# mit-han-lab/distrifuser

Hardware: NVIDIA H100
Metric: SDXL 50-step latency (ms/image) (lower is better)
Workload: dtype f16

## Files before the change

### distrifuser_b200/csrc/attention.cu

```cuda

#include "tc_ptx.cuh"

using namespace df;
using namespace df::tc;

namespace {

constexpr int BM = 128;
constexpr int BN = 128;
constexpr int HB = 64;
constexpr int NCONSUMER_WARPS = 8;
constexpr int NTHREADS = 32 * (NCONSUMER_WARPS + 1);
constexpr int WARP_TMA = NCONSUMER_WARPS;
constexpr uint32_t BLK_BYTES = BN * HB * 2;

template <int NBLK, int KSTAGES, int VSTAGES>
struct __align__(1024) SmemT {
  __half q[NBLK][BM * HB];
  __half k[KSTAGES][NBLK][BN * HB];
  __half v[VSTAGES][NBLK][BN * HB];
  uint64_t q_full, q_empty;
  uint64_t k_full[KSTAGES], k_empty[KSTAGES], v_full[VSTAGES], v_empty[VSTAGES];
  uint64_t sched_full[2];
  int sched_code[2];
  uint32_t ticket;
};
template <int NBLK> struct Cfg;
template <> struct Cfg<1> { static constexpr int KST = 3, VST = 2, SN = 128; };
template <> struct Cfg<2> { static constexpr int KST = 2, VST = 2, SN = 64; };
template <> struct Cfg<3> { static constexpr int KST = 2, VST = 1, SN = 64; };

struct Sched {
  int a, R, P;
  int dyn;
  int units;
};
constexpr int ITEM_END = -1;

__device__ __forceinline__ float2 ld_f2(const float2* p) {
  float2 r;
  asm volatile("ld.global.v2.f32 {%0, %1}, [%2];" : "=f"(r.x), "=f"(r.y) : "l"(p) : "memory");
  return r;
}

struct SegInfo {
  int32_t rank[DF_MAX_WORLD];
};

#ifndef DF_EMU_GROUPS
#define DF_EMU_GROUPS 3
#endif

template <int N>
__device__ __forceinline__ void wgmma_ss(float* d, uint64_t a_desc, uint64_t b_desc, uint32_t accumulate) {
  if constexpr (N == 64) wgmma_ss_n64(d, a_desc, b_desc, accumulate);
  else wgmma_ss_n128(d, a_desc, b_desc, accumulate);
}

template <int NBLK>
__global__ void __launch_bounds__(NTHREADS, 1)
fmha_fwd_kernel(const __grid_constant__ CUtensorMap tm_q, const __grid_constant__ CUtensorMap tm_kv_own,
                const CUtensorMap* __restrict__ kvmaps, df_comm_t comm, SegInfo segs, __half* __restrict__ out, int lq,
                int lseg, int heads, int d, int64_t o_pitch, int nseg, int own_seg, int idx, int wait_flags,
                float scale_log2, Sched sched, float* part_o, float2* part_ml, unsigned int* part_cnt, unsigned int* sched_ctr) {
  constexpr int KSTAGES = Cfg<NBLK>::KST, VSTAGES = Cfg<NBLK>::VST;
  constexpr uint32_t TILE_BYTES = NBLK * BLK_BYTES;
  constexpr int SN = Cfg<NBLK>::SN, NSUB = BN / SN;
  using Smem = SmemT<NBLK, KSTAGES, VSTAGES>;
  extern __shared__ __align__(1024) uint8_t smem_raw[];
  Smem& sm = *reinterpret_cast<Smem*>(smem_raw);
  if ((smem_u32(smem_raw) & 1023u) != 0) __trap();

  const int warp = threadIdx.x >> 5, lane = threadIdx.x & 31;
  const int nqt = (lq + BM - 1) / BM;
  const int tps = (lseg + BN - 1) / BN;
  const int T_all = nseg * tps;
  const int n_items = sched.a + ((int)blockIdx.x < sched.R * sched.P ? 1 : 0);
  auto decode = [&](int it, int& q0, int& head, int& bat, int& j_begin, int& T, int& slot, int& lo) {
    int u;
    if (sched.dyn) {
      u = it; j_begin = 0; T = T_all; slot = -1; lo = -1;
    } else if (it < sched.a) {
      u = it * (int)gridDim.x + (int)blockIdx.x; j_begin = 0; T = T_all; slot = -1; lo = -1;
    } else {
      lo = (int)blockIdx.x / sched.P;
      const int part = (int)blockIdx.x - lo * sched.P;
      u = sched.a * (int)gridDim.x + lo;
      j_begin = (int)((long long)part * T_all / sched.P);
      T = (int)((long long)(part + 1) * T_all / sched.P) - j_begin;
      slot = sched.P > 1 ? (int)blockIdx.x : -1;
    }
    const int qt = u % nqt, rest = u / nqt;
    head = rest % heads;
    bat = rest / heads;
    q0 = qt * BM;
  };

  if (threadIdx.x == 0) {
    mbar_init(&sm.q_full, 1);
    mbar_init(&sm.q_empty, NCONSUMER_WARPS);
    for (int s = 0; s < KSTAGES; ++s) { mbar_init(&sm.k_full[s], 1); mbar_init(&sm.k_empty[s], NCONSUMER_WARPS); }
    for (int s = 0; s < VSTAGES; ++s) { mbar_init(&sm.v_full[s], 1); mbar_init(&sm.v_empty[s], NCONSUMER_WARPS); }
    mbar_init(&sm.sched_full[0], 1);
    mbar_init(&sm.sched_full[1], 1);
    asm volatile("fence.mbarrier_init.release.cluster;" ::: "memory");
  }
  __syncthreads();
  pdl_wait();

  if (warp == WARP_TMA) {
    if (lane == 0) {
      prefetch_tmap(&tm_q);
      prefetch_tmap(&tm_kv_own);
      uint32_t rd = 0;
      if (nseg > 1) rd = comm.clock[1];
      int it_static = 0;
      auto draw = [&]() -> unsigned int {
        if (sched.dyn) return atomicAdd(sched_ctr, 1u);
        return (unsigned int)it_static++;
      };
      const unsigned int n_fresh = sched.dyn ? (unsigned int)sched.units : (unsigned int)n_items;
      unsigned int next_t = draw();
      uint32_t g = 0;
      for (uint32_t ui = 0;; ++ui) {
        int code = ITEM_END;
        if (next_t < n_fresh) {
          code = (int)next_t;
          next_t = draw();
        } else if (sched.dyn && next_t == n_fresh + gridDim.x - 1u) {
          *sched_ctr = 0u;
        }
        mbar_wait(&sm.q_empty, (ui & 1u) ^ 1u);
        *(volatile int*)&sm.sched_code[ui & 1u] = code;
        mbar_arrive(&sm.sched_full[ui & 1u]);
        if (code == ITEM_END) break;
        int q0, head, bat, j_begin, T, slot, lo;
        decode(code, q0, head, bat, j_begin, T, slot, lo);
        mbar_expect_tx(&sm.q_full, TILE_BYTES);
#pragma unroll
        for (int blk = 0; blk < NBLK; ++blk) tma_load_4d(sm.q[blk], &tm_q, &sm.q_full, blk * HB, head, q0, bat);
        int so = j_begin / tps, t = j_begin - so * tps;
        for (int j = 0; j < T; ++j, ++t, ++g) {
          if (t == tps) { t = 0; ++so; }
          int seg = own_seg + so;
          if (seg >= nseg) seg -= nseg;
          const void* map = &tm_kv_own;
          if (seg != own_seg) {
            const int r = segs.rank[seg];
            if ((t == 0 || j == 0) && wait_flags) {
              spin_until(flag_ptr(comm, comm.rank, idx, r), rd, comm.spin_timeout_ns);
              asm volatile("fence.proxy.async.global;" ::: "memory");
            }
            map = kvmaps + (size_t)(rd % DF_NBANKS) * comm.world + r;
          }
          const uint32_t ks = g % KSTAGES, vs = g % VSTAGES;
          mbar_wait(&sm.k_empty[ks], ((g / KSTAGES) & 1u) ^ 1u);
          mbar_expect_tx(&sm.k_full[ks], TILE_BYTES);
#pragma unroll
          for (int blk = 0; blk < NBLK; ++blk) tma_load_4d(sm.k[ks][blk], map, &sm.k_full[ks], blk * HB, head, t * BN, bat);
          mbar_wait(&sm.v_empty[vs], ((g / VSTAGES) & 1u) ^ 1u);
          mbar_expect_tx(&sm.v_full[vs], TILE_BYTES);
#pragma unroll
          for (int blk = 0; blk < NBLK; ++blk) tma_load_4d(sm.v[vs][blk], map, &sm.v_full[vs], blk * HB, heads + head, t * BN, bat);
        }
      }
    }
  } else {
    const int wg = warp >> 2;
    const int c4 = lane & 3;
    const int rowA = wg * 64 + (warp & 3) * 16 + (lane >> 2);
    const uint32_t q_base = smem_u32(sm.q) + wg * 64 * 128;
    uint32_t g = 0;
    for (uint32_t ui = 0;; ++ui) {
      mbar_wait(&sm.sched_full[ui & 1u], (ui >> 1) & 1u);
      const int code = *(volatile int*)&sm.sched_code[ui & 1u];
      if (code == ITEM_END) break;
      int q0, head, bat, j_begin, T, slot, lo;
      decode(code, q0, head, bat, j_begin, T, slot, lo);
      float nA = INFINITY, nB = INFINITY;
      float lA = 0.f, lB = 0.f;
      float o[NBLK * 32];
#pragma unroll
      for (int i = 0; i < NBLK * 32; ++i) o[i] = 0.f;
      mbar_wait(&sm.q_full, ui & 1u);
      int t = j_begin % tps;
      for (int j = 0; j < T; ++j, ++t, ++g) {
        if (t == tps) t = 0;
        const int valid = min(BN, lseg - t * BN);
        const uint32_t ks = g % KSTAGES, vs = g % VSTAGES;
#pragma unroll
        for (int sub = 0; sub < NSUB; ++sub) {
          float s[SN / 2];
          if (sub == 0) mbar_wait(&sm.k_full[ks], (g / KSTAGES) & 1u);
          const uint32_t k_addr = smem_u32(sm.k[ks]) + sub * SN * 128;
          wgmma_fence();
#pragma unroll
          for (int blk = 0; blk < NBLK; ++blk)
#pragma unroll
            for (int kk = 0; kk < HB / 16; ++kk)
              wgmma_ss<SN>(s, smem_desc(q_base + blk * BLK_BYTES + kk * 32, 16, 1024), smem_desc(k_addr + blk * BLK_BYTES + kk * 32, 16, 1024),
                           (blk | kk) > 0);
          wgmma_commit();
          wgmma_wait<0>();
          fence_regs<SN / 2>(s);
          if (sub == NSUB - 1) {
            __syncwarp();
            if (lane == 0) {
              mbar_arrive(&sm.k_empty[ks]);
              if (j + 1 == T) mbar_arrive(&sm.q_empty);
            }
          }
          const int vcols = valid - sub * SN;
          if (vcols < SN) {
#pragma unroll
            for (int i = 0; i < SN / 8; ++i)
#pragma unroll
              for (int k = 0; k < 2; ++k)
                if (8 * i + 2 * c4 + k >= vcols) { s[4 * i + k] = -INFINITY; s[4 * i + 2 + k] = -INFINITY; }
          }
          float mA0 = -INFINITY, mA1 = -INFINITY, mB0 = -INFINITY, mB1 = -INFINITY;
#pragma unroll
          for (int i = 0; i < SN / 8; i += 2) {
            mA0 = fmaxf(mA0, fmaxf(s[4 * i], s[4 * i + 1]));
            mB0 = fmaxf(mB0, fmaxf(s[4 * i + 2], s[4 * i + 3]));
            mA1 = fmaxf(mA1, fmaxf(s[4 * i + 4], s[4 * i + 5]));
            mB1 = fmaxf(mB1, fmaxf(s[4 * i + 6], s[4 * i + 7]));
          }
          float mA = fmaxf(mA0, mA1), mB = fmaxf(mB0, mB1);
          mA = fmaxf(mA, __shfl_xor_sync(0xffffffffu, mA, 1));
          mB = fmaxf(mB, __shfl_xor_sync(0xffffffffu, mB, 1));
          mA = fmaxf(mA, __shfl_xor_sync(0xffffffffu, mA, 2));
          mB = fmaxf(mB, __shfl_xor_sync(0xffffffffu, mB, 2));
          const float dA = fmaf(mA, scale_log2, nA), dB = fmaf(mB, scale_log2, nB);
          if (dA > 8.f) {
            const float alpha = ex2(-dA);
            nA = -mA * scale_log2; lA *= alpha;
#pragma unroll
            for (int i = 0; i < NBLK * 8; ++i) { o[4 * i] *= alpha; o[4 * i + 1] *= alpha; }
          }
          if (dB > 8.f) {
            const float alpha = ex2(-dB);
            nB = -mB * scale_log2; lB *= alpha;
#pragma unroll
            for (int i = 0; i < NBLK * 8; ++i) { o[4 * i + 2] *= alpha; o[4 * i + 3] *= alpha; }
          }
          uint32_t pk[SN / 4];
#pragma unroll
          for (int i = 0; i < SN / 8; ++i) {
            const int grp = sub * (SN / 8) + i;
            float e[4];
#pragma unroll
            for (int k = 0; k < 4; ++k) {
              const float x = fmaf(s[4 * i + k], scale_log2, k < 2 ? nA : nB);
              e[k] = ((grp * DF_EMU_GROUPS) / 16 != ((grp + 1) * DF_EMU_GROUPS) / 16) ? ex2_poly(x) : ex2(x);
            }
            lA += e[0] + e[1];
            lB += e[2] + e[3];
            pk[2 * i] = pack_h2(e[0], e[1]);
            pk[2 * i + 1] = pack_h2(e[2], e[3]);
          }
          if (sub == 0) mbar_wait(&sm.v_full[vs], (g / VSTAGES) & 1u);
          const uint32_t v_addr = smem_u32(sm.v[vs]) + sub * SN * 128;
          wgmma_fence();
#pragma unroll
          for (int kk = 0; kk < SN / 16; ++kk)
#pragma unroll
            for (int blk = 0; blk < NBLK; ++blk)
              wgmma_rs_n64(o + 32 * blk, pk + 4 * kk, smem_desc(v_addr + blk * BLK_BYTES + kk * 2048, 16384, 1024), 1u);
          wgmma_commit();
          wgmma_wait<0>();
          fence_regs<NBLK * 32>(o);
        }
        __syncwarp();
        if (lane == 0) mbar_arrive(&sm.v_empty[vs]);
      }
      lA += __shfl_xor_sync(0xffffffffu, lA, 1); lB += __shfl_xor_sync(0xffffffffu, lB, 1);
      lA += __shfl_xor_sync(0xffffffffu, lA, 2); lB += __shfl_xor_sync(0xffffffffu, lB, 2);
      const bool partial = slot >= 0;
      bool finish = !partial;
      float denA = lA, denB = lB;
      if (partial) {
        const int64_t prow = (int64_t)slot * BM + rowA;
        if (c4 == 0) { part_ml[prow] = make_float2(-nA, lA); part_ml[prow + 8] = make_float2(-nB, lB); }
#pragma unroll
        for (int i = 0; i < NBLK * 8; ++i) {
          const int col = 8 * i + 2 * c4;
          *reinterpret_cast<float2*>(part_o + prow * (NBLK * HB) + col) = make_float2(o[4 * i], o[4 * i + 1]);
          *reinterpret_cast<float2*>(part_o + (prow + 8) * (NBLK * HB) + col) = make_float2(o[4 * i + 2], o[4 * i + 3]);
        }
        __threadfence();
        asm volatile("bar.sync 1, 256;" ::: "memory");
        if (threadIdx.x == 0) {
          const unsigned int tk = atomicAdd(part_cnt + lo, 1u);
          sm.ticket = tk;
          if (tk == (unsigned int)sched.P - 1) part_cnt[lo] = 0;
        }
        asm volatile("bar.sync 1, 256;" ::: "memory");
        finish = sm.ticket == (unsigned int)sched.P - 1;
        if (finish) {
          __threadfence();
          const int s0 = lo * sched.P;
#pragma unroll
          for (int h = 0; h < 2; ++h) {
            const int64_t r = rowA + 8 * h;
            float m_max = -INFINITY;
            for (int pp = 0; pp < sched.P; ++pp) m_max = fmaxf(m_max, ld_f2(part_ml + (int64_t)(s0 + pp) * BM + r).x);
            float den = 0.f;
#pragma unroll
            for (int i = 0; i < NBLK * 8; ++i) { o[4 * i + 2 * h] = 0.f; o[4 * i + 2 * h + 1] = 0.f; }
            for (int pp = 0; pp < sched.P; ++pp) {
              const float2 ml = ld_f2(part_ml + (int64_t)(s0 + pp) * BM + r);
              const float w = ex2(ml.x - m_max);
              den = fmaf(w, ml.y, den);
              const float2* src = reinterpret_cast<const float2*>(part_o + ((int64_t)(s0 + pp) * BM + r) * (NBLK * HB));
#pragma unroll
              for (int i = 0; i < NBLK * 8; ++i) {
                const float2 v = ld_f2(src + 4 * i + c4);
                o[4 * i + 2 * h] = fmaf(w, v.x, o[4 * i + 2 * h]);
                o[4 * i + 2 * h + 1] = fmaf(w, v.y, o[4 * i + 2 * h + 1]);
              }
            }
            if (h == 0) denA = den; else denB = den;
          }
        }
      }
      if (finish) {
#pragma unroll
        for (int h = 0; h < 2; ++h) {
          const int row = rowA + 8 * h;
          if (q0 + row >= lq) continue;
          const float inv = 1.f / (h == 0 ? denA : denB);
          __half* dst = out + ((int64_t)bat * lq + q0 + row) * o_pitch + (int64_t)head * d;
#pragma unroll
          for (int i = 0; i < NBLK * 8; ++i) {
            const int col = 8 * i + 2 * c4;
            if (col < d)
              *reinterpret_cast<uint32_t*>(dst + col) = pack_h2(o[4 * i + 2 * h] * inv, o[4 * i + 2 * h + 1] * inv);
          }
        }
      }
    }
  }
}


int make_map(CUtensorMap* m, const void* base, int d, int nheads, int rows, int batch, int64_t pitch) {
  EncodeTiledFn enc = tensor_map_encoder();
  DF_REQUIRE(enc != nullptr, "cuTensorMapEncodeTiled is not available from this driver");
  cuuint64_t dims[4] = {(cuuint64_t)d, (cuuint64_t)nheads, (cuuint64_t)rows, (cuuint64_t)batch};
  cuuint64_t strides[3] = {(cuuint64_t)d * 2, (cuuint64_t)pitch * 2, (cuuint64_t)rows * pitch * 2};
  cuuint32_t box[4] = {HB, 1, BN, 1};
  cuuint32_t estr[4] = {1, 1, 1, 1};
  CUresult r = enc(m, CU_TENSOR_MAP_DATA_TYPE_FLOAT16, 4, const_cast<void*>(base), dims, strides, box, estr,
                   CU_TENSOR_MAP_INTERLEAVE_NONE, CU_TENSOR_MAP_SWIZZLE_128B, CU_TENSOR_MAP_L2_PROMOTION_L2_256B,
                   CU_TENSOR_MAP_FLOAT_OOB_FILL_NONE);
  DF_REQUIRE(r == CUDA_SUCCESS, "cuTensorMapEncodeTiled failed (%d): base=%p d=%d heads=%d rows=%d batch=%d pitch=%lld", (int)r,
             base, d, nheads, rows, batch, (long long)pitch);
  return 0;
}

}

extern "C" int df_attn_make_kvmaps(df_comm_t comm, uint64_t tensor_off, uint64_t slot_bytes, int b, int lseg, int heads,
                                   int d, void* maps_out, void* stream) {
  static_assert(sizeof(CUtensorMap) == DF_TENSORMAP_BYTES, "tensor map size");
  DF_REQUIRE(d % 8 == 0 && d >= 8 && d <= 192, "df_attn: head dim %d not supported (multiple of 8, <= 192)", d);
  DF_REQUIRE(slot_bytes >= (uint64_t)b * lseg * 2 * heads * d * 2, "df_attn_make_kvmaps: slot too small");
  CUtensorMap host[DF_NBANKS * DF_MAX_WORLD];
  memset(host, 0, sizeof(host));
  const int64_t pitch = 2 * (int64_t)heads * d;
  for (int k = 0; k < DF_NBANKS; ++k)
    for (int s = 0; s < comm.world; ++s) {
      const char* base = slot_ptr(comm, comm.rank, (uint32_t)k, tensor_off, slot_bytes, s);
      if (int rc = make_map(&host[k * comm.world + s], base, d, 2 * heads, lseg, b, pitch)) return rc;
    }
  DF_CHECK_CUDA(cudaMemcpyAsync(maps_out, host, sizeof(CUtensorMap) * DF_NBANKS * comm.world, cudaMemcpyHostToDevice,
                                (cudaStream_t)stream));
  DF_CHECK_CUDA(cudaStreamSynchronize((cudaStream_t)stream));
  return 0;
}

namespace {
#ifndef DF_MIN_PART_TILES
#define DF_MIN_PART_TILES 8
#endif
void plan_schedule(int b, int lq, int lseg, int nseg, int heads, int d, bool have_ws, int& grid, Sched& sc) {
  (void)d;
  const long long slots = sm_count();
  const long long units = (long long)((lq + BM - 1) / BM) * heads * b;
  const int t_all = nseg * ((lseg + BN - 1) / BN);
  sc.units = (int)units;
  if (units >= slots) {
    grid = (int)slots;
    sc.a = (int)(units / slots);
    sc.R = (int)(units % slots);
    sc.P = 1;
    sc.dyn = have_ws ? 1 : 0;
  } else {
    long long p = have_ws ? slots / units : 1;
    if (p > t_all / DF_MIN_PART_TILES) p = t_all / DF_MIN_PART_TILES;
    if (p < 1) p = 1;
    sc.a = 0; sc.R = (int)units; sc.P = (int)p; sc.dyn = 0;
    grid = (int)(units * p);
  }
}
constexpr size_t WS_HEADER = 1024;
size_t workspace_need(const Sched& sc, int d) {
  if (sc.P <= 1) return WS_HEADER;
  const size_t hd_pad = (size_t)((d + HB - 1) / HB) * HB;
  const size_t parts = (size_t)sc.R * sc.P;
  return WS_HEADER + 1024 + ((size_t)sc.R * sizeof(unsigned int) + 255) / 256 * 256 + parts * BM * sizeof(float2) + parts * BM * hd_pad * sizeof(float);
}
}

extern "C" size_t df_attn_workspace_bytes(int b, int lq, int lseg, int nseg, int heads, int d) {
  int grid;
  Sched sc;
  plan_schedule(b, lq, lseg, nseg, heads, d, true, grid, sc);
  return workspace_need(sc, d);
}

extern "C" int df_attn_fwd(df_comm_t comm, const void* q, const void* kv_own, void* out, const void* kvmaps, int b, int lq,
                           int lseg, int heads, int d, int64_t q_pitch, int64_t kv_pitch, int64_t o_pitch, int nseg,
                           int own_seg, const int32_t* seg_rank_host, int idx, int wait_flags, float scale, void* workspace,
                           size_t workspace_bytes, void* stream) {
  DF_REQUIRE(d % 8 == 0 && d >= 8 && d <= 192, "df_attn_fwd: head dim %d not supported (multiple of 8, <= 192)", d);
  DF_REQUIRE(nseg >= 1 && nseg <= DF_MAX_WORLD && own_seg >= 0 && own_seg < nseg, "df_attn_fwd: bad segment layout");
  DF_REQUIRE(nseg == 1 || kvmaps != nullptr, "df_attn_fwd: peer segments need tensor maps (df_attn_make_kvmaps)");
  DF_REQUIRE(q_pitch % 8 == 0 && kv_pitch % 8 == 0 && o_pitch % 8 == 0 && ((uintptr_t)q % 16) == 0 &&
                 ((uintptr_t)kv_own % 16) == 0 && ((uintptr_t)out % 16) == 0,
             "df_attn_fwd: q/kv/out must be 16-byte aligned with pitches multiple of 8");
  DF_REQUIRE(b >= 1 && lq >= 1 && lseg >= 1 && heads >= 1 && heads <= 65535 && b <= 65535, "df_attn_fwd: bad shape");
  CUtensorMap tq, tkv;
  if (int rc = make_map(&tq, q, d, heads, lq, b, q_pitch)) return rc;
  if (int rc = make_map(&tkv, kv_own, d, 2 * heads, lseg, b, kv_pitch)) return rc;
  SegInfo segs;
  for (int s = 0; s < DF_MAX_WORLD; ++s) segs.rank[s] = (s < nseg && seg_rank_host) ? seg_rank_host[s] : 0;
  const float sc = (scale > 0.f ? scale : 1.f / sqrtf((float)d)) * 1.4426950408889634f;
  const int nblk = (d + HB - 1) / HB;
  int grid_x;
  Sched sched;
  plan_schedule(b, lq, lseg, nseg, heads, d, true, grid_x, sched);
  if (workspace == nullptr || workspace_bytes < workspace_need(sched, d))
    plan_schedule(b, lq, lseg, nseg, heads, d, false, grid_x, sched);
  unsigned int* sched_ctr = sched.dyn ? (unsigned int*)workspace : nullptr;
  unsigned int* part_cnt = nullptr;
  float2* part_ml = nullptr;
  float* part_o = nullptr;
  if (sched.P > 1) {
    char* w = (char*)workspace + WS_HEADER;
    part_cnt = (unsigned int*)w;
    w += ((size_t)sched.R * sizeof(unsigned int) + 255) / 256 * 256;
    part_ml = (float2*)w;
    w += (size_t)sched.R * sched.P * BM * sizeof(float2);
    part_o = (float*)(((uintptr_t)w + 255) / 256 * 256);
  }
  dim3 grid((unsigned)grid_x, 1, 1);
#define DF_LAUNCH_FMHA(NB)                                                                                                  \
  {                                                                                                                          \
    static bool attr_set = false;                                                                                            \
    const size_t smem_bytes = sizeof(SmemT<NB, Cfg<NB>::KST, Cfg<NB>::VST>);                                                 \
    if (!attr_set) {                                                                                                         \
      DF_CHECK_CUDA(cudaFuncSetAttribute(fmha_fwd_kernel<NB>, cudaFuncAttributeMaxDynamicSharedMemorySize, (int)smem_bytes)); \
      attr_set = true;                                                                                                       \
    }                                                                                                                        \
    DF_CHECK_CUDA(launch_pdl(PDL_ATTN, fmha_fwd_kernel<NB>, grid, dim3(NTHREADS), smem_bytes, (cudaStream_t)stream, tq, tkv,           \
                             (const CUtensorMap*)kvmaps, comm, segs, (__half*)out, lq, lseg, heads, d, o_pitch, nseg,        \
                             own_seg, idx, wait_flags, sc, sched, part_o, part_ml, part_cnt, sched_ctr));                               \
  }
  if (nblk == 1) DF_LAUNCH_FMHA(1) else if (nblk == 2) DF_LAUNCH_FMHA(2) else DF_LAUNCH_FMHA(3)
#undef DF_LAUNCH_FMHA
  DF_CHECK_LAUNCH();
  return 0;
}
```

### distrifuser_b200/csrc/common.cuh

```cuda
#pragma once
#include <cuda.h>
#include <cuda_fp16.h>
#include <cuda_runtime.h>
#include <stdint.h>
#include <stdio.h>

#include "../../include/distrifuser_b200.h"

namespace df {

constexpr int kSmCount = 132;
int sm_count();

typedef CUresult (*EncodeTiledFn)(CUtensorMap*, CUtensorMapDataType, cuuint32_t, void*, const cuuint64_t*, const cuuint64_t*,
                                  const cuuint32_t*, const cuuint32_t*, CUtensorMapInterleave, CUtensorMapSwizzle,
                                  CUtensorMapL2promotion, CUtensorMapFloatOOBfill);
EncodeTiledFn tensor_map_encoder();

void set_error(const char* fmt, ...);

#define DF_CHECK_CUDA(expr)                                                              \
  do {                                                                                   \
    cudaError_t _e = (expr);                                                             \
    if (_e != cudaSuccess) {                                                             \
      df::set_error("%s:%d %s -> %s", __FILE__, __LINE__, #expr, cudaGetErrorString(_e)); \
      return 1;                                                                          \
    }                                                                                    \
  } while (0)

#define DF_REQUIRE(cond, ...)        \
  do {                               \
    if (!(cond)) {                   \
      df::set_error(__VA_ARGS__);    \
      return 2;                      \
    }                                \
  } while (0)

#define DF_CHECK_LAUNCH() DF_CHECK_CUDA(cudaGetLastError())

__device__ __forceinline__ uint32_t ld_acquire_sys(const uint32_t* p) {
  uint32_t v;
  asm volatile("ld.acquire.sys.global.u32 %0, [%1];" : "=r"(v) : "l"(p) : "memory");
  return v;
}
__device__ __forceinline__ void st_release_sys(uint32_t* p, uint32_t v) {
  asm volatile("st.release.sys.global.u32 [%0], %1;" ::"l"(p), "r"(v) : "memory");
}
__device__ __forceinline__ uint32_t ld_volatile_u32(const uint32_t* p) {
  uint32_t v;
  asm volatile("ld.volatile.global.u32 %0, [%1];" : "=r"(v) : "l"(p) : "memory");
  return v;
}
__device__ __forceinline__ bool epoch_reached(uint32_t flag, uint32_t want) { return (int32_t)(flag - want) >= 0; }

__device__ __forceinline__ uint64_t globaltimer_ns() {
  uint64_t t;
  asm volatile("mov.u64 %0, %globaltimer;" : "=l"(t));
  return t;
}
#ifndef DF_SPIN_TIMEOUT_NS
#define DF_SPIN_TIMEOUT_NS 30000000000ull
#endif
__device__ __forceinline__ void spin_until(const uint32_t* flag, uint32_t want, uint64_t timeout_ns = 0) {
  if (epoch_reached(ld_acquire_sys(flag), want)) return;
  if (timeout_ns == 0) timeout_ns = DF_SPIN_TIMEOUT_NS;
  const uint64_t t0 = globaltimer_ns();
  uint32_t polls = 0;
  while (!epoch_reached(ld_acquire_sys(flag), want)) {
    __nanosleep(64);
    if ((++polls & 1023u) == 0 && globaltimer_ns() - t0 > timeout_ns) {
      printf("distrifuser_b200: timeout waiting for flag %p (have %u, want %u)\n", (const void*)flag, ld_volatile_u32(flag), want);
      __trap();
    }
  }
}

__device__ __forceinline__ int4 ld_nc_v4(const void* p) {
  int4 r;
  asm volatile("ld.global.nc.L1::no_allocate.v4.s32 {%0,%1,%2,%3}, [%4];"
               : "=r"(r.x), "=r"(r.y), "=r"(r.z), "=r"(r.w)
               : "l"(p));
  return r;
}
__device__ __forceinline__ int4 ld_v4(const void* p) {
  int4 r;
  asm volatile("ld.global.v4.s32 {%0,%1,%2,%3}, [%4];" : "=r"(r.x), "=r"(r.y), "=r"(r.z), "=r"(r.w) : "l"(p));
  return r;
}
__device__ __forceinline__ void st_v4(void* p, const int4& v) {
  asm volatile("st.global.v4.s32 [%0], {%1,%2,%3,%4};" ::"l"(p), "r"(v.x), "r"(v.y), "r"(v.z), "r"(v.w) : "memory");
}

unsigned pdl_mask();
enum { PDL_ATTN = 1, PDL_ELEM = 2, PDL_GN = 4, PDL_GEMM = 8 };

__device__ __forceinline__ void pdl_wait() { asm volatile("griddepcontrol.wait;" ::: "memory"); }

template <typename... KArgs, typename... Args>
inline cudaError_t launch_pdl(unsigned family, void (*kernel)(KArgs...), dim3 grid, dim3 block, size_t smem, cudaStream_t st, Args... args) {
  cudaLaunchConfig_t cfg = {};
  cfg.gridDim = grid;
  cfg.blockDim = block;
  cfg.dynamicSmemBytes = smem;
  cfg.stream = st;
  cudaLaunchAttribute attr[1];
  attr[0].id = cudaLaunchAttributeProgrammaticStreamSerialization;
  attr[0].val.programmaticStreamSerializationAllowed = (pdl_mask() & family) ? 1 : 0;
  cfg.attrs = attr;
  cfg.numAttrs = 1;
  return cudaLaunchKernelEx(&cfg, kernel, static_cast<KArgs>(args)...);
}


__host__ __device__ __forceinline__ uint64_t slot_offset(const df_comm_t& c, uint32_t epoch, uint64_t tensor_off,
                                                         uint64_t slot_bytes, int src) {
  return (uint64_t)(epoch % DF_NBANKS) * c.bank_stride + tensor_off + (uint64_t)src * slot_bytes;
}
__host__ __device__ __forceinline__ char* slot_ptr(const df_comm_t& c, int rank, uint32_t epoch, uint64_t tensor_off,
                                                   uint64_t slot_bytes, int src) {
  return (char*)c.base[rank] + slot_offset(c, epoch, tensor_off, slot_bytes, src);
}

__device__ __forceinline__ uint32_t* flag_ptr(const df_comm_t& c, int member, int idx, int src) {
  return c.flags[member] + (size_t)idx * c.world + src;
}

__device__ __forceinline__ void stamp_flags(const df_comm_t& c, int idx, uint32_t mask, uint32_t epoch, int first = 0, int step = 1) {
  for (int p = first; p < c.world; p += step)
    if (mask >> p & 1) st_release_sys(flag_ptr(c, p, idx, c.rank), epoch);
}

__device__ __forceinline__ void wait_sources(const df_comm_t& c, int idx, uint32_t mask, uint32_t epoch) {
  const int s = threadIdx.x;
  if (s < c.world && (mask >> s & 1)) spin_until(flag_ptr(c, c.rank, idx, s), epoch, c.spin_timeout_ns);
  __syncthreads();
}

__device__ __forceinline__ uint32_t neighbour_mask(int up, int down) {
  return (up >= 0 ? 1u << up : 0u) | (down >= 0 ? 1u << down : 0u);
}

__device__ __forceinline__ void signal_when_last(const df_comm_t& c, unsigned int* ticket, unsigned int nctas, int idx,
                                                 uint32_t mask, uint32_t epoch) {
  __threadfence_system();
  __syncthreads();
  if (threadIdx.x == 0) {
    if (atomicAdd(ticket, 1u) == nctas - 1) {
      __threadfence();
      *ticket = 0;
      stamp_flags(c, idx, mask, epoch);
    }
  }
}

}
```

### distrifuser_b200/csrc/tc_ptx.cuh

```cuda
#pragma once
#include <cuda.h>

#include "common.cuh"

namespace df {
namespace tc {

__device__ __forceinline__ uint32_t smem_u32(const void* p) { return (uint32_t)__cvta_generic_to_shared(p); }

__device__ __forceinline__ void mbar_init(uint64_t* bar, uint32_t count) {
  asm volatile("mbarrier.init.shared::cta.b64 [%0], %1;" ::"r"(smem_u32(bar)), "r"(count));
}
__device__ __forceinline__ void mbar_expect_tx(uint64_t* bar, uint32_t bytes) {
  asm volatile("mbarrier.arrive.expect_tx.shared::cta.b64 _, [%0], %1;" ::"r"(smem_u32(bar)), "r"(bytes) : "memory");
}
__device__ __forceinline__ void mbar_arrive(uint32_t bar_addr) {
  asm volatile("mbarrier.arrive.shared::cta.b64 _, [%0];" ::"r"(bar_addr) : "memory");
}
__device__ __forceinline__ void mbar_arrive(uint64_t* bar) { mbar_arrive(smem_u32(bar)); }
#ifndef DF_TRYWAIT_HINT_NS
#define DF_TRYWAIT_HINT_NS 200000u
#endif
__device__ __forceinline__ bool mbar_try(uint32_t bar_addr, uint32_t parity) {
  uint32_t ok;
  asm volatile(
      "{\n\t.reg .pred p;\n\t"
      "mbarrier.try_wait.parity.shared::cta.b64 p, [%1], %2, %3;\n\t"
      "selp.u32 %0, 1, 0, p;\n\t}"
      : "=r"(ok)
      : "r"(bar_addr), "r"(parity), "r"(DF_TRYWAIT_HINT_NS)
      : "memory");
  return ok != 0;
}
__device__ __forceinline__ bool mbar_try(uint64_t* bar, uint32_t parity) { return mbar_try(smem_u32(bar), parity); }
__device__ __forceinline__ void mbar_wait(uint32_t bar, uint32_t parity) {
  if (mbar_try(bar, parity)) return;
  uint32_t polls = 0;
  uint64_t t0 = 0;
  while (!mbar_try(bar, parity)) {
    if ((++polls & 0x3FFu) == 0) {
      const uint64_t now = globaltimer_ns();
      if (t0 == 0) t0 = now;
      else if (now - t0 > 10000000000ull) {
#ifdef DF_MBAR_DEBUG
        printf("distrifuser_b200: mbarrier timeout (block %d,%d,%d thread %d bar@%u parity %u)\n", blockIdx.x, blockIdx.y, blockIdx.z,
               threadIdx.x, bar, parity);
#endif
        __trap();
      }
    }
  }
}

__device__ __forceinline__ void mbar_wait(uint64_t* bar, uint32_t parity) { mbar_wait(smem_u32(bar), parity); }

__device__ __forceinline__ void tma_load_4d(void* dst, const void* tmap, uint64_t* bar, int c0, int c1, int c2, int c3) {
  asm volatile(
      "cp.async.bulk.tensor.4d.shared::cluster.global.mbarrier::complete_tx::bytes [%0], [%1, {%3, %4, %5, %6}], [%2];"
      ::"r"(smem_u32(dst)), "l"((uint64_t)tmap), "r"(smem_u32(bar)), "r"(c0), "r"(c1), "r"(c2), "r"(c3)
      : "memory");
}
__device__ __forceinline__ void tma_load_2d(void* dst, const void* tmap, uint64_t* bar, int c0, int c1) {
  asm volatile(
      "cp.async.bulk.tensor.2d.shared::cluster.global.mbarrier::complete_tx::bytes [%0], [%1, {%3, %4}], [%2];"
      ::"r"(smem_u32(dst)), "l"((uint64_t)tmap), "r"(smem_u32(bar)), "r"(c0), "r"(c1)
      : "memory");
}
__device__ __forceinline__ void prefetch_tmap(const void* tmap) {
  asm volatile("prefetch.tensormap [%0];" ::"l"((uint64_t)tmap) : "memory");
}

__device__ __forceinline__ uint64_t smem_desc(uint32_t addr, uint32_t lbo_bytes, uint32_t sbo_bytes) {
  return (uint64_t)((addr & 0x3FFFFu) >> 4) | ((uint64_t)((lbo_bytes >> 4) & 0x3FFFu) << 16) |
         ((uint64_t)((sbo_bytes >> 4) & 0x3FFFu) << 32) | (1ull << 62);
}
__device__ __forceinline__ void wgmma_fence() { asm volatile("wgmma.fence.sync.aligned;" ::: "memory"); }
__device__ __forceinline__ void wgmma_commit() { asm volatile("wgmma.commit_group.sync.aligned;" ::: "memory"); }
template <int N>
__device__ __forceinline__ void wgmma_wait() { asm volatile("wgmma.wait_group.sync.aligned %0;" ::"n"(N) : "memory"); }
template <int N>
__device__ __forceinline__ void fence_regs(float* d) {
#pragma unroll
  for (int i = 0; i < N; ++i) asm volatile("" : "+f"(d[i])::"memory");
}

__device__ __forceinline__ void wgmma_ss_n64(float* d, uint64_t a_desc, uint64_t b_desc, uint32_t accumulate) {
  asm volatile(
      "{\n\t.reg .pred p;\n\tsetp.ne.b32 p, %34, 0;\n\t"
      "wgmma.mma_async.sync.aligned.m64n64k16.f32.f16.f16 {%0, %1, %2, %3, %4, %5, %6, %7, %8, %9, %10, %11, %12, %13, %14, %15, %16, %17, %18, %19, %20, %21, %22, %23, %24, %25, %26, %27, %28, %29, %30, %31}, %32, %33, p, 1, 1, 0, 0;\n\t}"
      : "+f"(d[0]), "+f"(d[1]), "+f"(d[2]), "+f"(d[3]), "+f"(d[4]), "+f"(d[5]), "+f"(d[6]), "+f"(d[7]), "+f"(d[8]), "+f"(d[9]), "+f"(d[10]), "+f"(d[11]), "+f"(d[12]), "+f"(d[13]), "+f"(d[14]), "+f"(d[15]), "+f"(d[16]), "+f"(d[17]), "+f"(d[18]), "+f"(d[19]), "+f"(d[20]), "+f"(d[21]), "+f"(d[22]), "+f"(d[23]), "+f"(d[24]), "+f"(d[25]), "+f"(d[26]), "+f"(d[27]), "+f"(d[28]), "+f"(d[29]), "+f"(d[30]), "+f"(d[31])
      : "l"(a_desc), "l"(b_desc), "r"(accumulate));
}
__device__ __forceinline__ void wgmma_ss_n128(float* d, uint64_t a_desc, uint64_t b_desc, uint32_t accumulate) {
  asm volatile(
      "{\n\t.reg .pred p;\n\tsetp.ne.b32 p, %66, 0;\n\t"
      "wgmma.mma_async.sync.aligned.m64n128k16.f32.f16.f16 {%0, %1, %2, %3, %4, %5, %6, %7, %8, %9, %10, %11, %12, %13, %14, %15, %16, %17, %18, %19, %20, %21, %22, %23, %24, %25, %26, %27, %28, %29, %30, %31, %32, %33, %34, %35, %36, %37, %38, %39, %40, %41, %42, %43, %44, %45, %46, %47, %48, %49, %50, %51, %52, %53, %54, %55, %56, %57, %58, %59, %60, %61, %62, %63}, %64, %65, p, 1, 1, 0, 0;\n\t}"
      : "+f"(d[0]), "+f"(d[1]), "+f"(d[2]), "+f"(d[3]), "+f"(d[4]), "+f"(d[5]), "+f"(d[6]), "+f"(d[7]), "+f"(d[8]), "+f"(d[9]), "+f"(d[10]), "+f"(d[11]), "+f"(d[12]), "+f"(d[13]), "+f"(d[14]), "+f"(d[15]), "+f"(d[16]), "+f"(d[17]), "+f"(d[18]), "+f"(d[19]), "+f"(d[20]), "+f"(d[21]), "+f"(d[22]), "+f"(d[23]), "+f"(d[24]), "+f"(d[25]), "+f"(d[26]), "+f"(d[27]), "+f"(d[28]), "+f"(d[29]), "+f"(d[30]), "+f"(d[31]), "+f"(d[32]), "+f"(d[33]), "+f"(d[34]), "+f"(d[35]), "+f"(d[36]), "+f"(d[37]), "+f"(d[38]), "+f"(d[39]), "+f"(d[40]), "+f"(d[41]), "+f"(d[42]), "+f"(d[43]), "+f"(d[44]), "+f"(d[45]), "+f"(d[46]), "+f"(d[47]), "+f"(d[48]), "+f"(d[49]), "+f"(d[50]), "+f"(d[51]), "+f"(d[52]), "+f"(d[53]), "+f"(d[54]), "+f"(d[55]), "+f"(d[56]), "+f"(d[57]), "+f"(d[58]), "+f"(d[59]), "+f"(d[60]), "+f"(d[61]), "+f"(d[62]), "+f"(d[63])
      : "l"(a_desc), "l"(b_desc), "r"(accumulate));
}

__device__ __forceinline__ void wgmma_ss_n160(float* d, uint64_t a_desc, uint64_t b_desc, uint32_t accumulate) {
  asm volatile(
      "{\n\t.reg .pred p;\n\tsetp.ne.b32 p, %82, 0;\n\t"
      "wgmma.mma_async.sync.aligned.m64n160k16.f32.f16.f16 {%0, %1, %2, %3, %4, %5, %6, %7, %8, %9, %10, %11, %12, %13, %14, %15, %16, %17, %18, %19, %20, %21, %22, %23, %24, %25, %26, %27, %28, %29, %30, %31, %32, %33, %34, %35, %36, %37, %38, %39, %40, %41, %42, %43, %44, %45, %46, %47, %48, %49, %50, %51, %52, %53, %54, %55, %56, %57, %58, %59, %60, %61, %62, %63, %64, %65, %66, %67, %68, %69, %70, %71, %72, %73, %74, %75, %76, %77, %78, %79}, %80, %81, p, 1, 1, 0, 0;\n\t}"
      : "+f"(d[0]), "+f"(d[1]), "+f"(d[2]), "+f"(d[3]), "+f"(d[4]), "+f"(d[5]), "+f"(d[6]), "+f"(d[7]), "+f"(d[8]), "+f"(d[9]), "+f"(d[10]), "+f"(d[11]), "+f"(d[12]), "+f"(d[13]), "+f"(d[14]), "+f"(d[15]), "+f"(d[16]), "+f"(d[17]), "+f"(d[18]), "+f"(d[19]), "+f"(d[20]), "+f"(d[21]), "+f"(d[22]), "+f"(d[23]), "+f"(d[24]), "+f"(d[25]), "+f"(d[26]), "+f"(d[27]), "+f"(d[28]), "+f"(d[29]), "+f"(d[30]), "+f"(d[31]), "+f"(d[32]), "+f"(d[33]), "+f"(d[34]), "+f"(d[35]), "+f"(d[36]), "+f"(d[37]), "+f"(d[38]), "+f"(d[39]), "+f"(d[40]), "+f"(d[41]), "+f"(d[42]), "+f"(d[43]), "+f"(d[44]), "+f"(d[45]), "+f"(d[46]), "+f"(d[47]), "+f"(d[48]), "+f"(d[49]), "+f"(d[50]), "+f"(d[51]), "+f"(d[52]), "+f"(d[53]), "+f"(d[54]), "+f"(d[55]), "+f"(d[56]), "+f"(d[57]), "+f"(d[58]), "+f"(d[59]), "+f"(d[60]), "+f"(d[61]), "+f"(d[62]), "+f"(d[63]), "+f"(d[64]), "+f"(d[65]), "+f"(d[66]), "+f"(d[67]), "+f"(d[68]), "+f"(d[69]), "+f"(d[70]), "+f"(d[71]), "+f"(d[72]), "+f"(d[73]), "+f"(d[74]), "+f"(d[75]), "+f"(d[76]), "+f"(d[77]), "+f"(d[78]), "+f"(d[79])
      : "l"(a_desc), "l"(b_desc), "r"(accumulate));
}

__device__ __forceinline__ void wgmma_ss_n256(float* d, uint64_t a_desc, uint64_t b_desc, uint32_t accumulate) {
  asm volatile(
      "{\n\t.reg .pred p;\n\tsetp.ne.b32 p, %130, 0;\n\t"
      "wgmma.mma_async.sync.aligned.m64n256k16.f32.f16.f16 {%0, %1, %2, %3, %4, %5, %6, %7, %8, %9, %10, %11, %12, %13, %14, %15, %16, %17, %18, %19, %20, %21, %22, %23, %24, %25, %26, %27, %28, %29, %30, %31, %32, %33, %34, %35, %36, %37, %38, %39, %40, %41, %42, %43, %44, %45, %46, %47, %48, %49, %50, %51, %52, %53, %54, %55, %56, %57, %58, %59, %60, %61, %62, %63, %64, %65, %66, %67, %68, %69, %70, %71, %72, %73, %74, %75, %76, %77, %78, %79, %80, %81, %82, %83, %84, %85, %86, %87, %88, %89, %90, %91, %92, %93, %94, %95, %96, %97, %98, %99, %100, %101, %102, %103, %104, %105, %106, %107, %108, %109, %110, %111, %112, %113, %114, %115, %116, %117, %118, %119, %120, %121, %122, %123, %124, %125, %126, %127}, %128, %129, p, 1, 1, 0, 0;\n\t}"
      : "+f"(d[0]), "+f"(d[1]), "+f"(d[2]), "+f"(d[3]), "+f"(d[4]), "+f"(d[5]), "+f"(d[6]), "+f"(d[7]), "+f"(d[8]), "+f"(d[9]), "+f"(d[10]), "+f"(d[11]), "+f"(d[12]), "+f"(d[13]), "+f"(d[14]), "+f"(d[15]), "+f"(d[16]), "+f"(d[17]), "+f"(d[18]), "+f"(d[19]), "+f"(d[20]), "+f"(d[21]), "+f"(d[22]), "+f"(d[23]), "+f"(d[24]), "+f"(d[25]), "+f"(d[26]), "+f"(d[27]), "+f"(d[28]), "+f"(d[29]), "+f"(d[30]), "+f"(d[31]), "+f"(d[32]), "+f"(d[33]), "+f"(d[34]), "+f"(d[35]), "+f"(d[36]), "+f"(d[37]), "+f"(d[38]), "+f"(d[39]), "+f"(d[40]), "+f"(d[41]), "+f"(d[42]), "+f"(d[43]), "+f"(d[44]), "+f"(d[45]), "+f"(d[46]), "+f"(d[47]), "+f"(d[48]), "+f"(d[49]), "+f"(d[50]), "+f"(d[51]), "+f"(d[52]), "+f"(d[53]), "+f"(d[54]), "+f"(d[55]), "+f"(d[56]), "+f"(d[57]), "+f"(d[58]), "+f"(d[59]), "+f"(d[60]), "+f"(d[61]), "+f"(d[62]), "+f"(d[63]), "+f"(d[64]), "+f"(d[65]), "+f"(d[66]), "+f"(d[67]), "+f"(d[68]), "+f"(d[69]), "+f"(d[70]), "+f"(d[71]), "+f"(d[72]), "+f"(d[73]), "+f"(d[74]), "+f"(d[75]), "+f"(d[76]), "+f"(d[77]), "+f"(d[78]), "+f"(d[79]), "+f"(d[80]), "+f"(d[81]), "+f"(d[82]), "+f"(d[83]), "+f"(d[84]), "+f"(d[85]), "+f"(d[86]), "+f"(d[87]), "+f"(d[88]), "+f"(d[89]), "+f"(d[90]), "+f"(d[91]), "+f"(d[92]), "+f"(d[93]), "+f"(d[94]), "+f"(d[95]), "+f"(d[96]), "+f"(d[97]), "+f"(d[98]), "+f"(d[99]), "+f"(d[100]), "+f"(d[101]), "+f"(d[102]), "+f"(d[103]), "+f"(d[104]), "+f"(d[105]), "+f"(d[106]), "+f"(d[107]), "+f"(d[108]), "+f"(d[109]), "+f"(d[110]), "+f"(d[111]), "+f"(d[112]), "+f"(d[113]), "+f"(d[114]), "+f"(d[115]), "+f"(d[116]), "+f"(d[117]), "+f"(d[118]), "+f"(d[119]), "+f"(d[120]), "+f"(d[121]), "+f"(d[122]), "+f"(d[123]), "+f"(d[124]), "+f"(d[125]), "+f"(d[126]), "+f"(d[127])
      : "l"(a_desc), "l"(b_desc), "r"(accumulate));
}

__device__ __forceinline__ void wgmma_rs_n64(float* d, const uint32_t* a, uint64_t b_desc, uint32_t accumulate) {
  asm volatile(
      "{\n\t.reg .pred p;\n\tsetp.ne.b32 p, %37, 0;\n\t"
      "wgmma.mma_async.sync.aligned.m64n64k16.f32.f16.f16 {%0, %1, %2, %3, %4, %5, %6, %7, %8, %9, %10, %11, %12, %13, %14, %15, %16, %17, %18, %19, %20, %21, %22, %23, %24, %25, %26, %27, %28, %29, %30, %31}, {%32, %33, %34, %35}, %36, p, 1, 1, 1;\n\t}"
      : "+f"(d[0]), "+f"(d[1]), "+f"(d[2]), "+f"(d[3]), "+f"(d[4]), "+f"(d[5]), "+f"(d[6]), "+f"(d[7]), "+f"(d[8]), "+f"(d[9]), "+f"(d[10]), "+f"(d[11]), "+f"(d[12]), "+f"(d[13]), "+f"(d[14]), "+f"(d[15]), "+f"(d[16]), "+f"(d[17]), "+f"(d[18]), "+f"(d[19]), "+f"(d[20]), "+f"(d[21]), "+f"(d[22]), "+f"(d[23]), "+f"(d[24]), "+f"(d[25]), "+f"(d[26]), "+f"(d[27]), "+f"(d[28]), "+f"(d[29]), "+f"(d[30]), "+f"(d[31])
      : "r"(a[0]), "r"(a[1]), "r"(a[2]), "r"(a[3]), "l"(b_desc), "r"(accumulate));
}


__device__ __forceinline__ float ex2(float x) {
  float y;
  asm("ex2.approx.ftz.f32 %0, %1;" : "=f"(y) : "f"(x));
  return y;
}
__device__ __forceinline__ float ex2_poly(float x) {
  x = fmaxf(x, -127.f);
  const float r = __fadd_rd(x, 12582912.f);
  const float f = x - (r - 12582912.f);
  float q = fmaf(f, 0.077119089663028717041015625f, 0.227564394474029541015625f);
  q = fmaf(q, f, 0.695146143436431884765625f);
  q = fmaf(q, f, 1.f);
  return __int_as_float(__float_as_int(q) + (__float_as_int(r) << 23));
}
__device__ __forceinline__ uint32_t pack_h2(float lo, float hi) {
  __half2 h = __floats2half2_rn(lo, hi);
  return *reinterpret_cast<uint32_t*>(&h);
}


}
}
```

Before: 2141.

## Overlap QK and PV wgmma with warpgroup ping-pong and register reallocation

Restructures the attention consumer loop so that the S=QK^T wgmma for the current tile is issued together with the PV wgmma of the previous tile. Softmax then overlaps with tensor-core work, and the rescaling of O is deferred until after the PV wait. It adds a ping-pong schedule between the two consumer warpgroups using named barriers, and expands the producer to a full warpgroup so setmaxnreg can shift registers to the consumers. K/V pipeline stages are deepened for the 1- and 2-block configs. The risks are higher register pressure, smem growth from the extra stages, and barrier ordering bugs.

```diff
diff --git a/distrifuser_b200/csrc/attention.cu b/distrifuser_b200/csrc/attention.cu
--- a/distrifuser_b200/csrc/attention.cu
+++ b/distrifuser_b200/csrc/attention.cu
@@ -10,8 +10,9 @@
 constexpr int BN = 128;
 constexpr int HB = 64;
 constexpr int NCONSUMER_WARPS = 8;
-constexpr int NTHREADS = 32 * (NCONSUMER_WARPS + 1);
+constexpr int NTHREADS = 32 * (NCONSUMER_WARPS + 4);
 constexpr int WARP_TMA = NCONSUMER_WARPS;
+constexpr int PRODUCER_REGS = 56, CONSUMER_REGS = 224;
 constexpr uint32_t BLK_BYTES = BN * HB * 2;
 
 template <int NBLK, int KSTAGES, int VSTAGES>
@@ -26,9 +27,10 @@
   uint32_t ticket;
 };
 template <int NBLK> struct Cfg;
-template <> struct Cfg<1> { static constexpr int KST = 3, VST = 2, SN = 128; };
-template <> struct Cfg<2> { static constexpr int KST = 2, VST = 2, SN = 64; };
-template <> struct Cfg<3> { static constexpr int KST = 2, VST = 1, SN = 64; };
+template <> struct Cfg<1> { static constexpr int KST = 4, VST = 4, SN = 128; static constexpr bool OVERLAP = true, PINGPONG = true; };
+template <> struct Cfg<2> { static constexpr int KST = 3, VST = 3, SN = 64; static constexpr bool OVERLAP = true, PINGPONG = true; };
+template <> struct Cfg<3> { static constexpr int KST = 2, VST = 1, SN = 64; static constexpr bool OVERLAP = false, PINGPONG = false; };
+constexpr int TURN_BAR = 2;
 
 struct Sched {
   int a, R, P;
@@ -66,6 +68,7 @@
   constexpr int KSTAGES = Cfg<NBLK>::KST, VSTAGES = Cfg<NBLK>::VST;
   constexpr uint32_t TILE_BYTES = NBLK * BLK_BYTES;
   constexpr int SN = Cfg<NBLK>::SN, NSUB = BN / SN;
+  constexpr bool OVERLAP = Cfg<NBLK>::OVERLAP, PINGPONG = Cfg<NBLK>::PINGPONG;
   using Smem = SmemT<NBLK, KSTAGES, VSTAGES>;
   extern __shared__ __align__(1024) uint8_t smem_raw[];
   Smem& sm = *reinterpret_cast<Smem*>(smem_raw);
@@ -108,8 +111,9 @@
   __syncthreads();
   pdl_wait();
 
-  if (warp == WARP_TMA) {
-    if (lane == 0) {
+  if (warp >= WARP_TMA) {
+    setmaxnreg_dec<PRODUCER_REGS>();
+    if (warp == WARP_TMA && lane == 0) {
       prefetch_tmap(&tm_q);
       prefetch_tmap(&tm_kv_own);
       uint32_t rd = 0;
@@ -148,7 +152,7 @@
           if (seg != own_seg) {
             const int r = segs.rank[seg];
             if ((t == 0 || j == 0) && wait_flags) {
-              spin_until(flag_ptr(comm, comm.rank, idx, r), rd, comm.spin_timeout_ns);
+              spin_until<false>(flag_ptr(comm, comm.rank, idx, r), rd, comm.spin_timeout_ns);
               asm volatile("fence.proxy.async.global;" ::: "memory");
             }
             map = kvmaps + (size_t)(rd % DF_NBANKS) * comm.world + r;
@@ -166,15 +170,30 @@
       }
     }
   } else {
+    setmaxnreg_inc<CONSUMER_REGS>();
     const int wg = warp >> 2;
     const int c4 = lane & 3;
     const int rowA = wg * 64 + (warp & 3) * 16 + (lane >> 2);
     const uint32_t q_base = smem_u32(sm.q) + wg * 64 * 128;
     uint32_t g = 0;
+    auto turn_begin = [&]() {
+      if constexpr (PINGPONG) {
+        if (wg == 0) named_bar_sync<TURN_BAR, 256>(); else named_bar_sync<TURN_BAR + 1, 256>();
+      }
+    };
+    auto turn_end = [&]() {
+      if constexpr (PINGPONG) {
+        if (wg == 0) named_bar_arrive<TURN_BAR + 1, 256>(); else named_bar_arrive<TURN_BAR, 256>();
+      }
+    };
+    if (PINGPONG && wg == 1) named_bar_arrive<TURN_BAR, 256>();
     for (uint32_t ui = 0;; ++ui) {
       mbar_wait(&sm.sched_full[ui & 1u], (ui >> 1) & 1u);
       const int code = *(volatile int*)&sm.sched_code[ui & 1u];
-      if (code == ITEM_END) break;
+      if (code == ITEM_END) {
+        if (PINGPONG && wg == 0) named_bar_sync<TURN_BAR, 256>();
+        break;
+      }
       int q0, head, bat, j_begin, T, slot, lo;
       decode(code, q0, head, bat, j_begin, T, slot, lo);
       float nA = INFINITY, nB = INFINITY;
@@ -182,6 +201,29 @@
       float o[NBLK * 32];
 #pragma unroll
       for (int i = 0; i < NBLK * 32; ++i) o[i] = 0.f;
+      float s[SN / 2];
+      uint32_t pk[SN / 4];
+      auto issue_s = [&](uint32_t ks, int sub) {
+        const uint32_t k_addr = smem_u32(sm.k[ks]) + sub * SN * 128;
+        wgmma_fence();
+#pragma unroll
+        for (int blk = 0; blk < NBLK; ++blk)
+#pragma unroll
+          for (int kk = 0; kk < HB / 16; ++kk)
+            wgmma_ss<SN>(s, smem_desc(q_base + blk * BLK_BYTES + kk * 32, 16, 1024), smem_desc(k_addr + blk * BLK_BYTES + kk * 32, 16, 1024),
+                         (blk | kk) > 0);
+        wgmma_commit();
+      };
+      auto issue_pv = [&](uint32_t vs, int sub) {
+        const uint32_t v_addr = smem_u32(sm.v[vs]) + sub * SN * 128;
+        wgmma_fence();
+#pragma unroll
+        for (int kk = 0; kk < SN / 16; ++kk)
+#pragma unroll
+          for (int blk = 0; blk < NBLK; ++blk)
+            wgmma_rs_n64(o + 32 * blk, pk + 4 * kk, smem_desc(v_addr + blk * BLK_BYTES + kk * 2048, 16384, 1024), 1u);
+        wgmma_commit();
+      };
       mbar_wait(&sm.q_full, ui & 1u);
       int t = j_begin % tps;
       for (int j = 0; j < T; ++j, ++t, ++g) {
@@ -190,18 +232,17 @@
         const uint32_t ks = g % KSTAGES, vs = g % VSTAGES;
 #pragma unroll
         for (int sub = 0; sub < NSUB; ++sub) {
-          float s[SN / 2];
           if (sub == 0) mbar_wait(&sm.k_full[ks], (g / KSTAGES) & 1u);
-          const uint32_t k_addr = smem_u32(sm.k[ks]) + sub * SN * 128;
-          wgmma_fence();
-#pragma unroll
-          for (int blk = 0; blk < NBLK; ++blk)
-#pragma unroll
-            for (int kk = 0; kk < HB / 16; ++kk)
-              wgmma_ss<SN>(s, smem_desc(q_base + blk * BLK_BYTES + kk * 32, 16, 1024), smem_desc(k_addr + blk * BLK_BYTES + kk * 32, 16, 1024),
-                           (blk | kk) > 0);
-          wgmma_commit();
-          wgmma_wait<0>();
+          const bool pv = OVERLAP && (j > 0 || sub > 0);
+          const int subp = sub > 0 ? sub - 1 : NSUB - 1;
+          const uint32_t gp = sub > 0 ? g : g - 1u, vsp = gp % VSTAGES;
+          if (pv && subp == 0) mbar_wait(&sm.v_full[vsp], (gp / VSTAGES) & 1u);
+          turn_begin();
+          issue_s(ks, sub);
+          if (pv) issue_pv(vsp, subp);
+          else if (OVERLAP) wgmma_commit();
+          turn_end();
+          wgmma_wait<OVERLAP ? 1 : 0>();
           fence_regs<SN / 2>(s);
           if (sub == NSUB - 1) {
             __syncwarp();
@@ -232,47 +273,66 @@
           mA = fmaxf(mA, __shfl_xor_sync(0xffffffffu, mA, 2));
           mB = fmaxf(mB, __shfl_xor_sync(0xffffffffu, mB, 2));
           const float dA = fmaf(mA, scale_log2, nA), dB = fmaf(mB, scale_log2, nB);
-          if (dA > 8.f) {
-            const float alpha = ex2(-dA);
-            nA = -mA * scale_log2; lA *= alpha;
-#pragma unroll
-            for (int i = 0; i < NBLK * 8; ++i) { o[4 * i] *= alpha; o[4 * i + 1] *= alpha; }
-          }
-          if (dB > 8.f) {
-            const float alpha = ex2(-dB);
-            nB = -mB * scale_log2; lB *= alpha;
-#pragma unroll
-            for (int i = 0; i < NBLK * 8; ++i) { o[4 * i + 2] *= alpha; o[4 * i + 3] *= alpha; }
-          }
-          uint32_t pk[SN / 4];
+          const bool moveA = dA > 8.f, moveB = dB > 8.f;
+          float alphaA = 1.f, alphaB = 1.f;
+          if (moveA) { alphaA = ex2(-dA); nA = -mA * scale_log2; lA *= alphaA; }
+          if (moveB) { alphaB = ex2(-dB); nB = -mB * scale_log2; lB *= alphaB; }
 #pragma unroll
           for (int i = 0; i < SN / 8; ++i) {
             const int grp = sub * (SN / 8) + i;
-            float e[4];
 #pragma unroll
             for (int k = 0; k < 4; ++k) {
               const float x = fmaf(s[4 * i + k], scale_log2, k < 2 ? nA : nB);
-              e[k] = ((grp * DF_EMU_GROUPS) / 16 != ((grp + 1) * DF_EMU_GROUPS) / 16) ? ex2_poly(x) : ex2(x);
+              s[4 * i + k] = ((grp * DF_EMU_GROUPS) / 16 != ((grp + 1) * DF_EMU_GROUPS) / 16) ? ex2_poly(x) : ex2(x);
             }
-            lA += e[0] + e[1];
-            lB += e[2] + e[3];
-            pk[2 * i] = pack_h2(e[0], e[1]);
-            pk[2 * i + 1] = pack_h2(e[2], e[3]);
-          }
-          if (sub == 0) mbar_wait(&sm.v_full[vs], (g / VSTAGES) & 1u);
-          const uint32_t v_addr = smem_u32(sm.v[vs]) + sub * SN * 128;
-          wgmma_fence();
-#pragma unroll
-          for (int kk = 0; kk < SN / 16; ++kk)
-#pragma unroll
-            for (int blk = 0; blk < NBLK; ++blk)
-              wgmma_rs_n64(o + 32 * blk, pk + 4 * kk, smem_desc(v_addr + blk * BLK_BYTES + kk * 2048, 16384, 1024), 1u);
-          wgmma_commit();
-          wgmma_wait<0>();
-          fence_regs<NBLK * 32>(o);
-        }
+            lA += s[4 * i] + s[4 * i + 1];
+            lB += s[4 * i + 2] + s[4 * i + 3];
+          }
+          if (OVERLAP) {
+            wgmma_wait<0>();
+            fence_regs<NBLK * 32>(o);
+          }
+          if (pv) {
+            if (subp == NSUB - 1) {
+              __syncwarp();
+              if (lane == 0) mbar_arrive(&sm.v_empty[vsp]);
+            }
+          }
+          if (moveA) {
+#pragma unroll
+            for (int i = 0; i < NBLK * 8; ++i) { o[4 * i] *= alphaA; o[4 * i + 1] *= alphaA; }
+          }
+          if (moveB) {
+#pragma unroll
+            for (int i = 0; i < NBLK * 8; ++i) { o[4 * i + 2] *= alphaB; o[4 * i + 3] *= alphaB; }
+          }
+#pragma unroll
+          for (int i = 0; i < SN / 8; ++i) {
+            pk[2 * i] = pack_h2(s[4 * i], s[4 * i + 1]);
+            pk[2 * i + 1] = pack_h2(s[4 * i + 2], s[4 * i + 3]);
+          }
+          if constexpr (!OVERLAP) {
+            if (sub == 0) mbar_wait(&sm.v_full[vs], (g / VSTAGES) & 1u);
+            issue_pv(vs, sub);
+            wgmma_wait<0>();
+            fence_regs<NBLK * 32>(o);
+            if (sub == NSUB - 1) {
+              __syncwarp();
+              if (lane == 0) mbar_arrive(&sm.v_empty[vs]);
+            }
+          }
+        }
+      }
+      if constexpr (OVERLAP) {
+        const uint32_t vsp = (g - 1u) % VSTAGES;
+        if (NSUB == 1) mbar_wait(&sm.v_full[vsp], ((g - 1u) / VSTAGES) & 1u);
+        turn_begin();
+        issue_pv(vsp, NSUB - 1);
+        turn_end();
+        wgmma_wait<0>();
+        fence_regs<NBLK * 32>(o);
         __syncwarp();
-        if (lane == 0) mbar_arrive(&sm.v_empty[vs]);
+        if (lane == 0) mbar_arrive(&sm.v_empty[vsp]);
       }
       lA += __shfl_xor_sync(0xffffffffu, lA, 1); lB += __shfl_xor_sync(0xffffffffu, lB, 1);
       lA += __shfl_xor_sync(0xffffffffu, lA, 2); lB += __shfl_xor_sync(0xffffffffu, lB, 2);
diff --git a/distrifuser_b200/csrc/common.cuh b/distrifuser_b200/csrc/common.cuh
--- a/distrifuser_b200/csrc/common.cuh
+++ b/distrifuser_b200/csrc/common.cuh
@@ -61,6 +61,7 @@
 #ifndef DF_SPIN_TIMEOUT_NS
 #define DF_SPIN_TIMEOUT_NS 30000000000ull
 #endif
+template <bool kReport = true>
 __device__ __forceinline__ void spin_until(const uint32_t* flag, uint32_t want, uint64_t timeout_ns = 0) {
   if (epoch_reached(ld_acquire_sys(flag), want)) return;
   if (timeout_ns == 0) timeout_ns = DF_SPIN_TIMEOUT_NS;
@@ -69,7 +70,8 @@
   while (!epoch_reached(ld_acquire_sys(flag), want)) {
     __nanosleep(64);
     if ((++polls & 1023u) == 0 && globaltimer_ns() - t0 > timeout_ns) {
-      printf("distrifuser_b200: timeout waiting for flag %p (have %u, want %u)\n", (const void*)flag, ld_volatile_u32(flag), want);
+      if constexpr (kReport)
+        printf("distrifuser_b200: timeout waiting for flag %p (have %u, want %u)\n", (const void*)flag, ld_volatile_u32(flag), want);
       __trap();
     }
   }
diff --git a/distrifuser_b200/csrc/tc_ptx.cuh b/distrifuser_b200/csrc/tc_ptx.cuh
--- a/distrifuser_b200/csrc/tc_ptx.cuh
+++ b/distrifuser_b200/csrc/tc_ptx.cuh
@@ -79,6 +79,14 @@
 template <int N>
 __device__ __forceinline__ void wgmma_wait() { asm volatile("wgmma.wait_group.sync.aligned %0;" ::"n"(N) : "memory"); }
 template <int N>
+__device__ __forceinline__ void setmaxnreg_dec() { asm volatile("setmaxnreg.dec.sync.aligned.u32 %0;" ::"n"(N)); }
+template <int N>
+__device__ __forceinline__ void setmaxnreg_inc() { asm volatile("setmaxnreg.inc.sync.aligned.u32 %0;" ::"n"(N)); }
+template <int ID, int COUNT>
+__device__ __forceinline__ void named_bar_sync() { asm volatile("bar.sync %0, %1;" ::"n"(ID), "n"(COUNT) : "memory"); }
+template <int ID, int COUNT>
+__device__ __forceinline__ void named_bar_arrive() { asm volatile("bar.arrive %0, %1;" ::"n"(ID), "n"(COUNT) : "memory"); }
+template <int N>
 __device__ __forceinline__ void fence_regs(float* d) {
 #pragma unroll
   for (int i = 0; i < N; ++i) asm volatile("" : "+f"(d[i])::"memory");
```

Result: faster. 2075 (median of 6 runs) (-3.1%).
